# interpreting-video-features/interpreting-video-features

Hardware: AMD Instinct MI355X
Metric: clips/sec full mask-search (I3D, 16f, 300 iters) (higher is better)
Workload: dtype f32 (each operand as 3 bf16 planes = 24 significand bits, 6 MFMA passes, f32 accumulate, f32 storage); 1 GPU; I3D perturbation mask search, 300 iters, synthetic clips [32,3,16,224,224] per GPU per step (BASELINE configs[1]); init_mask + search + reverse score + Grad-CAM; iters=300, frames=16, math=bf16x6

## Files before the change

### interpreting-video-features_amd/csrc/conv3d_halo.hip

```cpp
#include "conv3d_halo_impl.h"

namespace ivf {

template int conv_halo_launch_variant_am<AM_X3>(ConvKArgs& a, int v, hipStream_t s);
extern template int conv_halo_launch_variant_am<AM_X6>(ConvKArgs& a, int v, hipStream_t s);
extern template int conv_halo_launch_variant_am<AM_BF16>(ConvKArgs& a, int v, hipStream_t s);

int conv_halo_supported(const ConvKArgs& a) {
  if (a.sT != 1 || a.sH != 1 || a.sW != 1) return 0;
  if (a.kT * a.kH * a.kW <= 1 || a.kT > 4 || a.kH > 4 || a.kW > 4) return 0;
  if (a.Cin % 8) return 0;
  return 1;
}

int conv_halo_num_variants() { return HALO_NUM_VARIANTS; }

int conv_halo_launch_variant(ConvKArgs& a, int math, int v, hipStream_t s) {
  switch (math) {
    case IVF_MATH_BF16X3: return conv_halo_launch_variant_am<AM_X3>(a, v, s);
    case IVF_MATH_BF16X6: return conv_halo_launch_variant_am<AM_X6>(a, v, s);
    case IVF_MATH_BF16ACT: return conv_halo_launch_variant_am<AM_BF16>(a, v, s);
  }
  set_error("conv3d_halo: arithmetic mode %d has no LDS-halo kernel", math);
  return IVF_ERR_UNSUPPORTED;
}

int conv_halo_launch(ConvKArgs& a, int math, hipStream_t s) {
  static const int widths[5] = {192, 128, 96, 64, 32};
  int best = 32, best_cost = 1 << 30;
  for (int w : widths) {
    int cost = cdiv(a.Cout, w) * (w + 40);
    if (cost < best_cost) { best_cost = cost; best = w; }
  }
  const bool deep = a.To >= 4;
  if (math == IVF_MATH_BF16X6) {
    switch (best) {
      case 192: return conv_halo_launch_variant(a, math, deep ? 68 : 18, s);
      case 128: return conv_halo_launch_variant(a, math, deep ? 61 : 9, s);
      case 96: return conv_halo_launch_variant(a, math, deep ? 20 : 10, s);
      case 64: return conv_halo_launch_variant(a, math, deep ? 21 : 11, s);
      default: return conv_halo_launch_variant(a, math, deep ? 37 : 12, s);
    }
  }
  switch (best) {
    case 192: return conv_halo_launch_variant(a, math, deep ? 0 : 8, s);
    case 128: return conv_halo_launch_variant(a, math, deep ? 1 : 9, s);
    case 96: return conv_halo_launch_variant(a, math, deep ? 3 : 10, s);
    case 64: return conv_halo_launch_variant(a, math, deep ? 5 : 11, s);
    default: return conv_halo_launch_variant(a, math, deep ? 7 : 12, s);
  }
}

}
```

### interpreting-video-features_amd/csrc/conv3d_halo_impl.h

```cpp
#pragma once
#include <algorithm>
#include <type_traits>

#include "conv_common.h"

namespace ivf {

#ifdef IVF_HALO_STAMPS
static __device__ unsigned long long g_halo_stamps[8];
#define IVF_STAMP(var) const unsigned long long var = __builtin_amdgcn_s_memtime()
#define IVF_STAMP_RT(var) const unsigned long long var = __builtin_amdgcn_s_memrealtime()
#define IVF_STAMP_ADD(slot, t1, t0) \
  do { if (threadIdx.x == 0) atomicAdd(&g_halo_stamps[slot], (t1) - (t0)); } while (0)
#else
#define IVF_STAMP(var) do {} while (0)
#define IVF_STAMP_RT(var) do {} while (0)
#define IVF_STAMP_ADD(slot, t1, t0) do {} while (0)
#endif

__device__ __forceinline__ void tile_hw(int p, int hw_pitch, int* h, int* w) {
  const int b0 = p & 1, b1 = (p >> 1) & 1, b2 = (p >> 2) & 1, b3 = (p >> 3) & 1, b4 = (p >> 4) & 1;
  const int half = p >> 5;
  int hl, ww;
  if (hw_pitch == 10) {
    ww = b0 | (b2 << 1) | (b1 << 2);
    hl = b3 | (b4 << 1);
  } else if (hw_pitch == 11) {
    ww = b0 | (b2 << 1) | (b3 << 2);
    hl = b1 | (b4 << 1);
  } else {
    ww = p & 7;
    hl = (p >> 3) & 3;
  }
  *h = half * 4 + hl;
  *w = ww;
}

template <int TT, int TH, int TW>
__device__ __forceinline__ void box_pos(int row, int hw_pitch, int* t, int* h, int* w) {
  if constexpr (TT == 4 && TW == 8) {
    const int li = row & 31, q = li >> 2, ql = q & 3;
    const int sel = ((ql + 1) >> 1) & 1;
    *t = (q >> 2) ? 3 - sel : sel;
    *w = (ql >> 1) * 4 + (li & 3);
    *h = row >> 5;
  } else if constexpr (TH == 8 && TW == 8) {
    tile_hw(row & 63, hw_pitch, h, w);
    *t = row >> 6;
  } else {
    const int p = row % (TH * TW);
    *t = row / (TH * TW);
    *h = p / TW;
    *w = p % TW;
  }
}

template <int TT, int TH, int TW>
__host__ __device__ constexpr int halo_plane_rows(int HH, int HW) {
  int ps = HH * HW;
  if (TT == 4 && TW == 8) ps += (4 - ps % 8 + 8) % 8;
  return ps;
}

template <int AM, int TT, int BN, int WROWS, int WCOLS, int KS, int BKH, int TH, int TW, int TPS, bool DMA>
__global__ __launch_bounds__((TT * TH * TW / WROWS) * (BN / WCOLS) * KS * 64) void conv3d_halo_kernel(ConvKArgs a,
                                                                                                int tilesT,
                                                                                                int tilesH,
                                                                                                int tilesW) {
  constexpr int BM = TT * TH * TW;
  constexpr int NPA = OpPlanes<AM>::A, NPB = OpPlanes<AM>::B;
  static_assert(BM % WROWS == 0 && WROWS % 32 == 0 && BN % WCOLS == 0 && WCOLS % 32 == 0, "tile");
  static_assert((KS * BN * (BKH / 8)) % 64 == 0, "weight-stream slots must fill whole waves");
  constexpr int WM = BM / WROWS, WN = BN / WCOLS;
  constexpr int NT = WM * WN * KS * 64;
  constexpr int TM = WROWS / 32, TN = WCOLS / 32;
  constexpr int ROWB = (BKH + 8) * 2;
  constexpr int ROWB_B = DMA ? BKH * 2 : ROWB;
  static_assert(!DMA || BKH == 32, "the LDS-DMA weight stream is written for 32-channel chunks");
  constexpr int G4 = BKH / 4;
  constexpr int G8 = BKH / 8;
  constexpr int BLOADS = (TPS * KS * BN * G8 + NT - 1) / NT;

  extern __shared__ __attribute__((aligned(16))) unsigned char smem[];
  IVF_STAMP(st_begin);
  IVF_STAMP_RT(rt_begin);
  const int HT = TT + a.kT - 1, HH = TH + a.kH - 1, HW = TW + a.kW - 1;
  const int PS = halo_plane_rows<TT, TH, TW>(HH, HW);
  const int HR = HT * PS;
  unsigned char* a_hi = smem;
  const size_t APL = (size_t)HR * ROWB;
  unsigned char* b_base = smem + (size_t)NPA * HR * ROWB;
  int* rowoff = reinterpret_cast<int*>(b_base + (size_t)2 * NPB * TPS * KS * BN * ROWB_B);

  const int tid = threadIdx.x;
  const int lane = tid & 63;
  const int wave = __builtin_amdgcn_readfirstlane(tid >> 6);
  const int wk = wave / (WM * WN);
  const int wm = (wave % (WM * WN)) / WN, wn = wave % WN;
  const int li = lane & 31, lh = lane >> 5;

  int tile = xcd_remap(blockIdx.x, gridDim.x);
  const int nt = tile % a.ntiles;
  tile /= a.ntiles;
  const int tw = tile % tilesW;
  tile /= tilesW;
  const int th = tile % tilesH;
  tile /= tilesH;
  const int tt = tile % tilesT;
  const int b = tile / tilesT;
  const int t0 = tt * TT, h0 = th * TH, w0 = tw * TW;
  const int n0 = nt * BN;

  int arow[TM];
#pragma unroll
  for (int i = 0; i < TM; ++i) {
    int r = wm * WROWS + i * 32 + li;
    int pt, ph, pw;
    box_pos<TT, TH, TW>(r, HW, &pt, &ph, &pw);
    arow[i] = pt * PS + ph * HW + pw;
  }
  const int ntaps = a.kT * a.kH * a.kW;
  const int ntg = (ntaps + KS - 1) / KS;
  const int nsteps = (ntg + TPS - 1) / TPS;
  const int khw = a.kH * a.kW;
  for (int row = tid; row < HR; row += NT) {
    int ht = row / PS;
    int rem = row - ht * PS;
    int hh = rem / HW;
    int hw = rem - hh * HW;
    int ti = t0 - a.pT + ht, hi = h0 - a.pH + hh, wi = w0 - a.pW + hw;
    bool ok = hh < HH && (unsigned)ti < (unsigned)a.Ti && (unsigned)hi < (unsigned)a.Hi && (unsigned)wi < (unsigned)a.Wi;
    rowoff[row] = ok ? ((b * a.Ti + ti) * a.Hi + hi) * a.Wi + wi : -1;
  }

  f32x16 acc[TM][TN];
#pragma unroll
  for (int i = 0; i < TM; ++i)
#pragma unroll
    for (int j = 0; j < TN; ++j)
#pragma unroll
      for (int r = 0; r < 16; ++r) acc[i][j][r] = 0.f;

  constexpr int PF = 3;
  typedef unsigned int u32x4 __attribute__((ext_vector_type(4)));
  u32x4 rb[PF][NPB][BLOADS] = {};
  int b_src[BLOADS];
  int b_dst[BLOADS];
  int b_tap[BLOADS];
  int b_c[BLOADS];
#pragma unroll
  for (int q = 0; q < BLOADS; ++q) {
    const int idx = tid + q * NT;
    const int sub = idx / (KS * BN * G8);
    const int r1 = idx - sub * (KS * BN * G8);
    const int grp = r1 / (BN * G8);
    const int rem = r1 - grp * (BN * G8);
    const int row = BKH == 32 ? perm8(rem / G8) : rem / G8, g2 = rem % G8;
    const int n = min(n0 + row, a.Cout - 1);
    b_src[q] = sub < TPS ? n * a.ldw : 0;
    b_dst[q] = sub < TPS ? ((sub * KS + grp) * NPB * BN + row) * ROWB_B + 16 * g2 : -1;
    b_tap[q] = sub < TPS ? sub + grp * ntg : 0;
    b_c[q] = 8 * g2;
  }
  auto load_b = [&](int slot, int step, int c0) __attribute__((always_inline)) {
    const int s0 = min(step, nsteps - 1) * TPS;
#pragma unroll
    for (int q = 0; q < BLOADS; ++q) {
      const int tap = min(s0 + b_tap[q], ntaps - 1);
      int c = c0 + b_c[q];
      c = c < a.Cin ? c : 0;
      const unsigned short* p = a.wbf + (size_t)(b_src[q] + tap * a.Cin + c);
      if (b_dst[q] >= 0) {
#pragma unroll
        for (int pl = 0; pl < NPB; ++pl) rb[slot][pl][q] = *reinterpret_cast<const u32x4*>(p + pl * a.w_lo_off);
      }
    }
  };
  auto store_b = [&](int slot, int buf) __attribute__((always_inline)) {
    unsigned char* bb = b_base + (size_t)buf * (TPS * KS * NPB * BN * ROWB_B);
#pragma unroll
    for (int q = 0; q < BLOADS; ++q) {
      if (b_dst[q] >= 0) {
#pragma unroll
        for (int pl = 0; pl < NPB; ++pl) *reinterpret_cast<u32x4*>(bb + b_dst[q] + pl * BN * ROWB_B) = rb[slot][pl][q];
      }
    }
  };
  int g_kw, g_kh, g_toff;
  {
    const int tap0 = wk * ntg;
    const int kt = tap0 / khw;
    const int rem = tap0 - kt * khw;
    g_kh = rem / a.kW;
    g_kw = rem - g_kh * a.kW;
    g_toff = (kt * PS + g_kh * HW + g_kw) * ROWB;
  }
  int t_kw = 0, t_kh = 0, t_off = 0;
  auto tap_advance = [&]() __attribute__((always_inline)) {
    t_off += ROWB;
    if (++t_kw == a.kW) {
      t_kw = 0;
      t_off += (HW - a.kW) * ROWB;
      if (++t_kh == a.kH) {
        t_kh = 0;
        t_off += (PS - a.kH * HW) * ROWB;
      }
    }
  };
  int abase[TM];
#pragma unroll
  for (int i = 0; i < TM; ++i) abase[i] = arow[i] * ROWB + 16 * lh;
  auto b_off = [&](int j, int ks) __attribute__((always_inline)) {
    const int row = wn * WCOLS + j * 32 + li;
    if constexpr (DMA) return row * ROWB_B + 16 * ((2 * ks + lh) ^ ((row >> 2) & 3));
    else return row * ROWB_B + ks * 32 + 16 * lh;
  };
  constexpr int NP = TPS * KS * NPB * BN * (BKH / 8), NI = NP / 64, NWV = NT / 64, MAXI = (NI + NWV - 1) / NWV;
  int d_base[MAXI], d_tap[MAXI], d_c[MAXI];
  if constexpr (DMA) {
#pragma unroll
    for (int k = 0; k < MAXI; ++k) {
      const int p = (wave + k * NWV) * 64 + lane;
      const int slot = p % G8, row = (p / G8) % BN, plane = (p / (G8 * BN)) % NPB;
      const int grp = (p / (G8 * BN * NPB)) % KS, sb = p / (G8 * BN * NPB * KS);
      d_base[k] = plane * (int)a.w_lo_off + min(n0 + row, a.Cout - 1) * a.ldw;
      d_tap[k] = sb + grp * ntg;
      d_c[k] = 8 * (slot ^ ((row >> 2) & 3));
    }
  }
  auto dma_b = [&](int step, int buf, int c0) __attribute__((always_inline)) {
    if constexpr (DMA) {
#pragma unroll
      for (int k = 0; k < MAXI; ++k) {
        if (wave + k * NWV >= NI) continue;
        const int tap = min(step * TPS + d_tap[k], ntaps - 1);
        int c = c0 + d_c[k];
        c = c < a.Cin ? c : 0;
        const unsigned short* g = a.wbf + (size_t)(d_base[k] + tap * a.Cin + c);
        unsigned char* dst = b_base + (size_t)buf * (TPS * KS * NPB * BN * ROWB_B) + (size_t)(wave + k * NWV) * 1024;
        __builtin_amdgcn_global_load_lds((const __attribute__((address_space(1))) void*)g,
                                         (__attribute__((address_space(3))) void*)dst, 16, 0, 0);
      }
    }
  };
  constexpr int NKS = BKH / 16;
  constexpr bool PIPELINED = (TM == 1 && TN == 1);
  auto mma_tap = [&](int step, int buf, int nks) __attribute__((always_inline)) {
    const int lt0 = step * TPS;
    const int nsub = min(TPS, min(ntg - lt0, ntaps - wk * ntg - lt0));
    if (nsub <= 0) return;
    const unsigned char* bstep = b_base + (size_t)(buf * TPS * KS + wk) * NPB * BN * ROWB_B;
    if constexpr (PIPELINED) {
      bf16x8 fa[2][NPA], fb[2][NPB];
      auto issue = [&](int slot, int sub, int ks) __attribute__((always_inline)) {
        const int aoff = abase[0] + t_off + ks * 32;
        const unsigned char* bh = bstep + (size_t)sub * KS * NPB * BN * ROWB_B + b_off(0, ks);
#pragma unroll
        for (int pl = 0; pl < NPA; ++pl) fa[slot][pl] = *reinterpret_cast<const bf16x8*>(a_hi + pl * APL + aoff);
#pragma unroll
        for (int pl = 0; pl < NPB; ++pl) fb[slot][pl] = *reinterpret_cast<const bf16x8*>(bh + (size_t)pl * BN * ROWB_B);
      };
      issue(0, 0, 0);
#pragma unroll
      for (int u = 0; u < TPS * NKS; ++u) {
        if (u / NKS < nsub) {
          if (u + 1 < TPS * NKS && (u + 1) / NKS < nsub) {
            if ((u + 1) % NKS == 0) tap_advance();
            issue((u + 1) & 1, (u + 1) / NKS, (u + 1) % NKS);
          }
          mma_planes<AM>(fa[u & 1], fb[u & 1], acc[0][0]);
          __builtin_amdgcn_sched_group_barrier(0x100, NPA + NPB, 0);
          __builtin_amdgcn_sched_group_barrier(0x008, AM == AM_X6 ? 6 : (AM == AM_BF16 ? 2 : 3), 0);
        }
      }
      tap_advance();
    } else {
#pragma unroll
      for (int sub = 0; sub < TPS; ++sub) {
        if (sub >= nsub) break;
        const unsigned char* bh = bstep + (size_t)sub * KS * NPB * BN * ROWB_B;
        for (int ks = 0; ks < nks; ++ks) {
          bf16x8 fa[TM][NPA];
#pragma unroll
          for (int i = 0; i < TM; ++i) {
            const int off = abase[i] + t_off + ks * 32;
#pragma unroll
            for (int pl = 0; pl < NPA; ++pl) fa[i][pl] = *reinterpret_cast<const bf16x8*>(a_hi + pl * APL + off);
          }
#pragma unroll
          for (int j = 0; j < TN; ++j) {
            const int off = b_off(j, ks);
            bf16x8 fb[NPB];
#pragma unroll
            for (int pl = 0; pl < NPB; ++pl) fb[pl] = *reinterpret_cast<const bf16x8*>(bh + (size_t)pl * BN * ROWB_B + off);
#pragma unroll
            for (int i = 0; i < TM; ++i) mma_planes<AM>(fa[i], fb, acc[i][j]);
          }
        }
        tap_advance();
      }
    }
  };

  constexpr int NSTG = 4;
  float4 stg[NSTG];
  const int ngroups = BKH == 32 ? ((HR + 7) & ~7) * G4 : HR * G4;
  int stage_base = 0;
  auto stage_load = [&](int c0) __attribute__((always_inline)) {
#pragma unroll
    for (int u = 0; u < NSTG; ++u) {
      int idx = stage_base + u * NT + tid;
      float4 v = make_float4(0.f, 0.f, 0.f, 0.f);
      if (idx < ngroups) {
        int row = BKH == 32 ? perm8(idx / G4) : idx / G4, g = idx % G4;
        if (row >= HR) row = -1;
        int c = c0 + 4 * g;
        int pos = row >= 0 ? rowoff[row] : -1;
        if (pos >= 0 && c < a.Cin) v = load_act4<AM>(a.in, (size_t)pos * a.in_ld + a.in_coff + c);
      }
      stg[u] = v;
    }
  };
  auto stage_store = [&]() __attribute__((always_inline)) {
#pragma unroll
    for (int u = 0; u < NSTG; ++u) {
      int idx = stage_base + u * NT + tid;
      const int srow = BKH == 32 ? perm8(idx / G4) : idx / G4;
      if (idx < ngroups && srow < HR) {
        stage_planes<AM>(a_hi + srow * ROWB + 8 * (idx % G4), APL, stg[u]);
      }
    }
  };
  __syncthreads();

  for (int c0 = 0; c0 < a.Cin; c0 += BKH) {
    if constexpr (!DMA) {
      load_b(0, 0, c0);
      load_b(1, 1, c0);
      load_b(2, 2, c0);
    }
    __syncthreads();
    dma_b(0, 0, c0);
    IVF_STAMP(st_s0);
    for (stage_base = 0; stage_base < ngroups; stage_base += NSTG * NT) {
      stage_load(c0);
      stage_store();
    }
    stage_base = 0;
    __builtin_amdgcn_s_waitcnt(0x0F70);
    if constexpr (!DMA) store_b(0, 0);
    __syncthreads();
    IVF_STAMP(st_s1);
    IVF_STAMP_ADD(1, st_s1, st_s0);

    const int cw = min(BKH, a.Cin - c0);
    const int nks = (cw + 15) >> 4;
    t_kw = g_kw, t_kh = g_kh, t_off = g_toff;
    auto tap_body = [&](auto U, int tap0) __attribute__((always_inline)) {
      constexpr int u = decltype(U)::value;
      const int tap = tap0 + u;
      load_b(u, tap + PF, c0);
      if (tap < nsteps) mma_tap(tap, tap & 1, nks);
      store_b((u + 1) % PF, (tap + 1) & 1);
      __syncthreads();
    };
    static_assert(PF == 3, "tap loop is unrolled by hand for a 3-deep ring");
    if constexpr (DMA) {
      for (int tap = 0; tap < nsteps; ++tap) {
        if (tap + 1 < nsteps) dma_b(tap + 1, (tap + 1) & 1, c0);
        mma_tap(tap, tap & 1, nks);
        asm volatile("s_waitcnt vmcnt(0)" ::: "memory");
        __syncthreads();
      }
    } else {
      for (int tap0 = 0; tap0 < nsteps; tap0 += PF) {
        tap_body(std::integral_constant<int, 0>{}, tap0);
        tap_body(std::integral_constant<int, 1>{}, tap0);
        tap_body(std::integral_constant<int, 2>{}, tap0);
      }
    }
    IVF_STAMP(st_s2);
    IVF_STAMP_ADD(2, st_s2, st_s1);
  }
  IVF_STAMP(st_loop_end);

  if constexpr (KS == 2) {
    float* red = reinterpret_cast<float*>(smem);
    const int slot = (wm * WN + wn) * TM * TN;
    if (wk == 1) {
#pragma unroll
      for (int i = 0; i < TM; ++i)
#pragma unroll
        for (int j = 0; j < TN; ++j)
#pragma unroll
          for (int r = 0; r < 16; ++r) red[((slot + i * TN + j) * 16 + r) * 64 + lane] = acc[i][j][r];
    }
    __syncthreads();
    if (wk == 0) {
#pragma unroll
      for (int i = 0; i < TM; ++i)
#pragma unroll
        for (int j = 0; j < TN; ++j)
#pragma unroll
          for (int r = 0; r < 16; ++r) acc[i][j][r] += red[((slot + i * TN + j) * 16 + r) * 64 + lane];
    }
    __syncthreads();
  }

  if (TH == 8 && TW == 8 && BN == 32 && a.d2s && a.Cout == 32 && a.bsT == 2 && a.bsH == 2 && a.bsW == 2 && !a.accumulate && !a.relu &&
      a.dC == 4 && (a.out_ld & 3) == 0 && (a.out_coff & 3) == 0) {
    float* ot = reinterpret_cast<float*>(smem);
    if (wk == 0) {
      const int n = wn * WCOLS + li;
      const int par = n >> 2, c = n & 3;
      const int pt = par >> 2, ph = (par >> 1) & 1, pw = par & 1;
#pragma unroll
      for (int i = 0; i < TM; ++i)
#pragma unroll
        for (int r = 0; r < 16; ++r) {
          const int row = wm * WROWS + i * 32 + (r & 3) + 8 * (r >> 2) + 4 * lh;
          int bt, bh, bw;
          box_pos<TT, TH, TW>(row, HW, &bt, &bh, &bw);
          const int tt2 = 2 * bt + pt, hh2 = 2 * bh + ph, ww2 = 2 * bw + pw;
          ot[((tt2 * 16 + hh2) * 16 + ww2) * 4 + c] = acc[i][0][r];
        }
    }
    __syncthreads();
    for (int p = tid; p < 2 * TT * 256; p += NT) {
      const int t = 2 * t0 + (p >> 8), h = 2 * h0 + ((p >> 4) & 15), w = 2 * w0 + (p & 15);
      if (t < a.dT && h < a.dH && w < a.dW)
        *reinterpret_cast<float4*>(a.out + ((size_t)((b * a.dT + t) * a.dH + h) * a.dW + w) * a.out_ld + a.out_coff) =
            *reinterpret_cast<const float4*>(ot + (size_t)p * 4);
    }
    IVF_STAMP(st_end_d2s);
    IVF_STAMP_RT(rt_end_d2s);
    IVF_STAMP_ADD(5, rt_end_d2s, rt_begin);
    IVF_STAMP_ADD(3, st_end_d2s, st_loop_end);
    IVF_STAMP_ADD(0, st_end_d2s, st_begin);
    IVF_STAMP_ADD(4, st_begin + 1, st_begin);
    return;
  }
  if (wk != 0) return;

  conv_epilogue<AM, TM, TN>(
      a, acc,
      [&](int row) {
        int pt, ph, pw;
        box_pos<TT, TH, TW>(row, HW, &pt, &ph, &pw);
        int t = t0 + pt, h = h0 + ph, w = w0 + pw;
        if (t >= a.To || h >= a.Ho || w >= a.Wo) return -1;
        return ((b * a.To + t) * a.Ho + h) * a.Wo + w;
      },
      wm * WROWS, n0 + wn * WCOLS, li, lh);
  IVF_STAMP(st_end);
  IVF_STAMP_RT(rt_end);
  IVF_STAMP_ADD(5, rt_end, rt_begin);
  IVF_STAMP_ADD(3, st_end, st_loop_end);
  IVF_STAMP_ADD(0, st_end, st_begin);
  IVF_STAMP_ADD(4, st_begin + 1, st_begin);
}

#if defined(IVF_HALO_STAMPS) && defined(IVF_HALO_STAMPS_OWNER)
}
extern "C" int ivf_debug_halo_stamps(unsigned long long* out8, int reset) {
  IVF_CHECK_HIP(hipMemcpyFromSymbol(out8, HIP_SYMBOL(ivf::g_halo_stamps), 8 * sizeof(unsigned long long)));
  if (reset) {
    unsigned long long z[8] = {0};
    IVF_CHECK_HIP(hipMemcpyToSymbol(HIP_SYMBOL(ivf::g_halo_stamps), z, sizeof(z)));
  }
  return IVF_OK;
}
namespace ivf {
#endif

template <int AM, int TT, int BN, int WROWS, int WCOLS, int KS = 1, int BKH = 32, int TH = 8, int TW = 8, int TPS = 1, bool DMA = false>
static int launch_halo(ConvKArgs& a, int variant_id, hipStream_t s) {
  constexpr int NPA = OpPlanes<AM>::A, NPB = OpPlanes<AM>::B;
  constexpr int NT = (TT * TH * TW / WROWS) * (BN / WCOLS) * KS * 64;
  constexpr int ROWB = (BKH + 8) * 2;
  constexpr int ROWB_B = DMA ? BKH * 2 : ROWB;
  const int HR = (TT + a.kT - 1) * halo_plane_rows<TT, TH, TW>(TH + a.kH - 1, TW + a.kW - 1);
  size_t shm = (size_t)NPA * HR * ROWB + (size_t)2 * TPS * KS * NPB * BN * ROWB_B + (size_t)HR * sizeof(int);
  if (KS == 2) shm = std::max(shm, (size_t)TT * TH * TW * BN * 4);
  if (a.d2s) shm = std::max(shm, (size_t)2 * TT * 256 * 4 * sizeof(float));
  if (shm > 160 * 1024) {
    set_error("conv3d_halo: %zu bytes of LDS needed", shm);
    return IVF_ERR_UNSUPPORTED;
  }
  static LdsAttrOnce once;
  IVF_PROPAGATE(raise_lds_limit(reinterpret_cast<const void*>(&conv3d_halo_kernel<AM, TT, BN, WROWS, WCOLS, KS, BKH, TH, TW, TPS, DMA>), 160 * 1024, once));
  const int tilesT = cdiv(a.To, TT), tilesH = cdiv(a.Ho, TH), tilesW = cdiv(a.Wo, TW);
  a.ntiles = cdiv(a.Cout, BN);
  a.mtiles = a.B * tilesT * tilesH * tilesW;
  dim3 grid(a.mtiles * a.ntiles);
  prof_name(IVF_CONV_HALO_BASE + variant_id, "conv3d_halo_kernel<%d,%d,%d,%d,%d,%d,%d,%d,%d,%d,%s>", AM, TT, BN, WROWS, WCOLS, KS,
            BKH, TH, TW, TPS, DMA ? "true" : "false");
  const bool timed = prof_begin(s, IVF_CONV_HALO_BASE + variant_id);
  hipLaunchKernelGGL((conv3d_halo_kernel<AM, TT, BN, WROWS, WCOLS, KS, BKH, TH, TW, TPS, DMA>), grid, dim3(NT), shm, s, a, tilesT, tilesH, tilesW);
  if (timed) prof_end(s);
  IVF_CHECK_LAUNCH();
  return IVF_OK;
}


constexpr int HALO_NUM_VARIANTS = 70;

template <int AM, int TT, int BN, int KS, int BKH, int TH, int TW, int TPS, bool DMA>
constexpr bool halo_variant_built() {
  constexpr int ROWB = (BKH + 8) * 2, ROWB_B = DMA ? BKH * 2 : ROWB;
  constexpr int HH = TH + 2, HW = TW + 2;
  constexpr int PS = HH * HW + ((TT == 4 && TW == 8) ? (4 - (HH * HW) % 8 + 8) % 8 : 0);
  constexpr long HR = (long)(TT + 2) * PS;
  constexpr long shm = OpPlanes<AM>::A * HR * ROWB + 2L * TPS * KS * OpPlanes<AM>::B * BN * ROWB_B + HR * 4;
  return shm <= 160 * 1024;
}
template <int AM, int TT, int BN, int WROWS, int WCOLS, int KS = 1, int BKH = 32, int TH = 8, int TW = 8, int TPS = 1, bool DMA = false>
static int launch_halo_if(ConvKArgs& a, int variant_id, hipStream_t s) {
  if constexpr (halo_variant_built<AM, TT, BN, KS, BKH, TH, TW, TPS, DMA>()) {
    return launch_halo<AM, TT, BN, WROWS, WCOLS, KS, BKH, TH, TW, TPS, DMA>(a, variant_id, s);
  } else {
    set_error("conv3d_halo: variant %d needs more than 160 KB of LDS in this arithmetic mode", variant_id);
    return IVF_ERR_UNSUPPORTED;
  }
}

template <int AM>
int conv_halo_launch_variant_am(ConvKArgs& a, int v, hipStream_t s) {
  switch (v) {
    case 0: return launch_halo_if<AM, 4, 192, 32, 96>(a, 0, s);
    case 1: return launch_halo_if<AM, 4, 128, 64, 64>(a, 1, s);
    case 2: return launch_halo_if<AM, 4, 128, 32, 64>(a, 2, s);
    case 3: return launch_halo_if<AM, 4, 96, 32, 96>(a, 3, s);
    case 4: return launch_halo_if<AM, 4, 64, 32, 64>(a, 4, s);
    case 5: return launch_halo_if<AM, 4, 64, 64, 64, 2>(a, 5, s);
    case 6: return launch_halo_if<AM, 4, 32, 32, 32>(a, 6, s);
    case 7: return launch_halo_if<AM, 4, 32, 64, 32, 2>(a, 7, s);
    case 8: return launch_halo_if<AM, 2, 192, 32, 96>(a, 8, s);
    case 9: return launch_halo_if<AM, 2, 128, 32, 64>(a, 9, s);
    case 10: return launch_halo_if<AM, 2, 96, 32, 96>(a, 10, s);
    case 11: return launch_halo_if<AM, 2, 64, 32, 64>(a, 11, s);
    case 12: return launch_halo_if<AM, 2, 32, 32, 32>(a, 12, s);
    case 13: return launch_halo_if<AM, 2, 64, 64, 64, 2>(a, 13, s);
    case 14: return launch_halo_if<AM, 2, 128, 64, 64>(a, 14, s);
    case 15: return launch_halo_if<AM, 4, 64, 32, 64, 2>(a, 15, s);
    case 16: return launch_halo_if<AM, 4, 96, 32, 96, 2>(a, 16, s);
    case 17: return launch_halo_if<AM, 4, 32, 32, 32, 2>(a, 17, s);
    case 18: return launch_halo_if<AM, 2, 192, 32, 96, 1, 16>(a, 18, s);
    case 19: return launch_halo_if<AM, 2, 128, 32, 64, 1, 16>(a, 19, s);
    case 20: return launch_halo_if<AM, 4, 96, 32, 96, 1, 16>(a, 20, s);
    case 21: return launch_halo_if<AM, 4, 64, 32, 64, 1, 16>(a, 21, s);
    case 22: return launch_halo_if<AM, 2, 96, 32, 96, 1, 16>(a, 22, s);
    case 23: return launch_halo_if<AM, 4, 192, 32, 96, 1, 32, 4, 14>(a, 23, s);
    case 24: return launch_halo_if<AM, 4, 128, 32, 64, 1, 32, 4, 14>(a, 24, s);
    case 25: return launch_halo_if<AM, 4, 96, 32, 96, 1, 32, 4, 14>(a, 25, s);
    case 26: return launch_halo_if<AM, 4, 64, 32, 64, 1, 32, 4, 14>(a, 26, s);
    case 27: return launch_halo_if<AM, 4, 32, 32, 32, 1, 32, 4, 14>(a, 27, s);
    case 28: return launch_halo_if<AM, 4, 64, 32, 32, 1, 32, 4, 14>(a, 28, s);
    case 29: return launch_halo_if<AM, 4, 32, 32, 32, 2, 32, 4, 14>(a, 29, s);
    case 30: return launch_halo_if<AM, 4, 128, 32, 128, 1, 32, 4, 14>(a, 30, s);
    case 31: return launch_halo_if<AM, 2, 32, 64, 32, 2, 16>(a, 31, s);
    case 32: return launch_halo_if<AM, 2, 32, 32, 32, 2, 16>(a, 32, s);
    case 33: return launch_halo_if<AM, 2, 32, 32, 32, 1, 16>(a, 33, s);
    case 34: return launch_halo_if<AM, 2, 64, 32, 64, 2, 16>(a, 34, s);
    case 35: return launch_halo_if<AM, 2, 64, 64, 64, 2, 16>(a, 35, s);
    case 36: return launch_halo_if<AM, 4, 32, 64, 32, 2, 16>(a, 36, s);
    case 37: return launch_halo_if<AM, 4, 32, 32, 32, 2, 16>(a, 37, s);
    case 38: return launch_halo_if<AM, 4, 32, 32, 32, 2, 16, 8, 8, 4>(a, 38, s);
    case 39: return launch_halo_if<AM, 4, 32, 64, 32, 2, 16, 8, 8, 4>(a, 39, s);
    case 40: return launch_halo_if<AM, 4, 32, 32, 32, 2, 16, 8, 8, 2>(a, 40, s);
    case 41: return launch_halo_if<AM, 2, 32, 32, 32, 2, 32, 8, 8, 2>(a, 41, s);
    case 42: return launch_halo_if<AM, 4, 64, 32, 64, 1, 16, 8, 8, 2>(a, 42, s);
    case 43: return launch_halo_if<AM, 4, 64, 32, 64, 1, 32, 8, 8, 2>(a, 43, s);
    case 44: return launch_halo_if<AM, 4, 32, 32, 32, 1, 16, 8, 8, 4>(a, 44, s);
    case 45: return launch_halo_if<AM, 4, 96, 32, 96, 1, 16, 8, 8, 2>(a, 45, s);
    case 46: return launch_halo_if<AM, 4, 32, 32, 32, 2, 32, 8, 8, 2>(a, 46, s);
    case 47: return launch_halo_if<AM, 4, 64, 32, 64, 1, 32, 4, 14, 2>(a, 47, s);
    case 48: return launch_halo_if<AM, 4, 192, 32, 96, 1, 32, 7, 8>(a, 48, s);
    case 49: return launch_halo_if<AM, 4, 128, 32, 64, 1, 32, 7, 8>(a, 49, s);
    case 50: return launch_halo_if<AM, 4, 96, 32, 96, 1, 16, 7, 8>(a, 50, s);
    case 51: return launch_halo_if<AM, 4, 64, 32, 64, 1, 16, 7, 8>(a, 51, s);
    case 52: return launch_halo_if<AM, 4, 192, 32, 96, 1, 32, 8, 8, 1, true>(a, 52, s);
    case 53: return launch_halo_if<AM, 4, 192, 32, 96, 1, 32, 4, 14, 1, true>(a, 53, s);
    case 54: return launch_halo_if<AM, 4, 128, 32, 64, 1, 32, 4, 14, 1, true>(a, 54, s);
    case 55: return launch_halo_if<AM, 4, 128, 32, 64, 1, 32, 8, 8, 1, true>(a, 55, s);
    case 56: return launch_halo_if<AM, 4, 32, 32, 32, 2, 32, 8, 8, 1, true>(a, 56, s);
    case 57: return launch_halo_if<AM, 4, 128, 32, 64, 1, 32, 7, 8, 1, true>(a, 57, s);
    case 58: return launch_halo_if<AM, 4, 96, 32, 96, 1, 32, 8, 8, 1, true>(a, 58, s);
    case 59: return launch_halo_if<AM, 4, 64, 32, 64, 1, 32, 8, 8, 1, true>(a, 59, s);
    case 60: return launch_halo_if<AM, 4, 192, 32, 96, 1, 16>(a, 60, s);
    case 61: return launch_halo_if<AM, 4, 128, 32, 64, 1, 16>(a, 61, s);
    case 62: return launch_halo_if<AM, 4, 192, 32, 96, 1, 16, 4, 14>(a, 62, s);
    case 63: return launch_halo_if<AM, 4, 128, 32, 64, 1, 16, 4, 14>(a, 63, s);
    case 64: return launch_halo_if<AM, 4, 96, 32, 96, 1, 16, 4, 14>(a, 64, s);
    case 65: return launch_halo_if<AM, 4, 64, 32, 64, 1, 16, 4, 14>(a, 65, s);
    case 66: return launch_halo_if<AM, 4, 192, 32, 96, 1, 16, 7, 8>(a, 66, s);
    case 67: return launch_halo_if<AM, 4, 128, 32, 64, 1, 16, 7, 8>(a, 67, s);
    case 68: return launch_halo_if<AM, 4, 192, 64, 96, 1, 16>(a, 68, s);
    case 69: return launch_halo_if<AM, 4, 128, 64, 64, 1, 16>(a, 69, s);
  }
  set_error("conv3d_halo: unknown variant %d", v);
  return IVF_ERR_BAD_ARG;
}

}
```

### interpreting-video-features_amd/csrc/ivf_common.hip

```cpp
#include <cstring>

#include "ivf_common.h"

namespace ivf {
static thread_local char g_err[512] = "";
void set_error(const char* fmt, ...) {
  va_list ap;
  va_start(ap, fmt);
  vsnprintf(g_err, sizeof(g_err), fmt, ap);
  va_end(ap);
}
}

extern "C" const char* ivf_last_error(void) { return ivf::g_err; }
extern "C" int ivf_version(void) { return 301; }

#include <vector>
namespace ivf {
struct Prof {
  bool enabled = false, active = false;
  int every = 1;
  size_t cap = 0, used = 0;
  std::vector<hipEvent_t> ev;
  std::vector<int> variant;
  std::vector<int> site;
  std::vector<double> flops;
  double next_flops = 0.0;
  int next_site = -1;
};
static Prof g_prof;
static char g_prof_names[IVF_PROFILE_CLASSES][96];
void prof_name(int variant, const char* fmt, ...) {
  if (variant < 0 || variant >= IVF_PROFILE_CLASSES) return;
  va_list ap;
  va_start(ap, fmt);
  vsnprintf(g_prof_names[variant], sizeof(g_prof_names[variant]), fmt, ap);
  va_end(ap);
}
void prof_set_iteration(int it) { g_prof.active = g_prof.enabled && it >= 0 && (it % g_prof.every == 0); }
void prof_set_flops(double f) { g_prof.next_flops = f; }
void prof_set_site(int site) { g_prof.next_site = site; }
bool prof_begin(hipStream_t s, int variant) {
  Prof& p = g_prof;
  if (!p.active || p.used >= p.cap) return false;
  if (p.ev.size() < 2 * (p.used + 1)) {
    hipEvent_t a, b;
    if (hipEventCreate(&a) != hipSuccess || hipEventCreate(&b) != hipSuccess) return false;
    p.ev.push_back(a);
    p.ev.push_back(b);
  }
  p.variant.resize(p.used + 1);
  p.site.resize(p.used + 1);
  p.flops.resize(p.used + 1);
  p.variant[p.used] = variant;
  p.site[p.used] = p.next_site;
  p.flops[p.used] = p.next_flops;
  (void)hipEventRecord(p.ev[2 * p.used], s);
  return true;
}
void prof_end(hipStream_t s) {
  Prof& p = g_prof;
  (void)hipEventRecord(p.ev[2 * p.used + 1], s);
  p.used++;
}
}

extern "C" int ivf_profile_enable(int every, int max_launches) {
  IVF_CHECK_ARG(every >= 1 && max_launches > 0, "profile_enable: bad args");
  ivf::g_prof.enabled = true;
  ivf::g_prof.active = false;
  ivf::g_prof.every = every;
  ivf::g_prof.cap = (size_t)max_launches;
  ivf::g_prof.used = 0;
  return IVF_OK;
}

extern "C" int ivf_profile_disable(void) {
  ivf::g_prof.enabled = false;
  ivf::g_prof.active = false;
  return IVF_OK;
}

extern "C" const char* ivf_profile_class_name(int cls) {
  return (cls >= 0 && cls < IVF_PROFILE_CLASSES) ? ivf::g_prof_names[cls] : "";
}

extern "C" int ivf_profile_collect_sites(double* kernel_ms, long long* launches, double* flops, int* variant,
                                         int max_sites) {
  IVF_CHECK_ARG(kernel_ms && launches && flops && variant && max_sites > 0, "profile_collect_sites: bad args");
  ivf::Prof& p = ivf::g_prof;
  for (int v = 0; v < max_sites; ++v) { kernel_ms[v] = 0.0; launches[v] = 0; flops[v] = 0.0; variant[v] = -1; }
  for (size_t i = 0; i < p.used; ++i) {
    const int st = p.site[i];
    if (st < 0 || st >= max_sites) continue;
    IVF_CHECK_HIP(hipEventSynchronize(p.ev[2 * i + 1]));
    float ms = 0.f;
    IVF_CHECK_HIP(hipEventElapsedTime(&ms, p.ev[2 * i], p.ev[2 * i + 1]));
    kernel_ms[st] += ms;
    launches[st] += 1;
    flops[st] += p.flops[i];
    variant[st] = p.variant[i];
  }
  return IVF_OK;
}

extern "C" int ivf_profile_collect(double* kernel_ms, long long* launches, double* flops) {
  IVF_CHECK_ARG(kernel_ms && launches && flops, "profile_collect: null pointer");
  ivf::Prof& p = ivf::g_prof;
  for (int v = 0; v < IVF_PROFILE_CLASSES; ++v) { kernel_ms[v] = 0.0; launches[v] = 0; flops[v] = 0.0; }
  for (size_t i = 0; i < p.used; ++i) {
    IVF_CHECK_HIP(hipEventSynchronize(p.ev[2 * i + 1]));
    float ms = 0.f;
    IVF_CHECK_HIP(hipEventElapsedTime(&ms, p.ev[2 * i], p.ev[2 * i + 1]));
    int v = p.variant[i];
    if (v < 0 || v >= IVF_PROFILE_CLASSES) continue;
    kernel_ms[v] += ms;
    launches[v] += 1;
    flops[v] += p.flops[i];
  }
  p.used = 0;
  return IVF_OK;
}
```

Baseline: 3.926 clips/s.

## Add raster-row halo conv variant for 3x3x3 convs on 14x14 maps

Adds a new conv3d halo kernel mode (RP=15) that tiles the output as a flat run of 256 consecutive output positions in raster order. The input halo is staged as a padded 15x15-pitch raster window, so each tap becomes a constant row offset and unpadded LDS rows are used. The dispatcher routes bf16x6 3x3x3 padding-1 convs on 13-14 spatial maps with Cout >= 2*Cin to this variant. The aim is to remove the wasted work and halo overhead that 8x8 box tiles incur on 14x14 maps. In exchange it stages a larger, irregular halo window per block and skips the LDS row padding, which may add bank conflicts.

Result: no change. 3.934 clips/s, median of 6 (+0.2%).

```diff
diff --git a/interpreting-video-features_amd/csrc/conv3d_halo.hip b/interpreting-video-features_amd/csrc/conv3d_halo.hip
--- a/interpreting-video-features_amd/csrc/conv3d_halo.hip
+++ b/interpreting-video-features_amd/csrc/conv3d_halo.hip
@@ -34,6 +34,9 @@
   }
   const bool deep = a.To >= 4;
   if (math == IVF_MATH_BF16X6) {
+    if (a.kT == 3 && a.kH == 3 && a.kW == 3 && a.pT == 1 && a.pH == 1 && a.pW == 1 && !a.d2s && a.Ho >= 13 && a.Ho <= 14 &&
+        a.Wo >= 13 && a.Wo <= 14 && a.Cin >= 144 && a.Cout >= 2 * a.Cin)
+      return conv_halo_launch_variant(a, math, 70, s);
     switch (best) {
       case 192: return conv_halo_launch_variant(a, math, deep ? 68 : 18, s);
       case 128: return conv_halo_launch_variant(a, math, deep ? 61 : 9, s);
diff --git a/interpreting-video-features_amd/csrc/conv3d_halo_impl.h b/interpreting-video-features_amd/csrc/conv3d_halo_impl.h
--- a/interpreting-video-features_amd/csrc/conv3d_halo_impl.h
+++ b/interpreting-video-features_amd/csrc/conv3d_halo_impl.h
@@ -62,7 +62,23 @@
   return ps;
 }
 
-template <int AM, int TT, int BN, int WROWS, int WCOLS, int KS, int BKH, int TH, int TW, int TPS, bool DMA>
+template <int RP>
+__host__ __device__ inline int raster_x(int m, int T, int H, int W) {
+  const int w = m % W;
+  const int r1 = m / W;
+  const int h = r1 % H;
+  const int r2 = r1 / H;
+  const int t = r2 % T, b = r2 / T;
+  return (b * (T + 1) + t + 1) * RP * RP + (h + 1) * RP + (w + 1);
+}
+template <int RP>
+inline int raster_window_bound(int BM, int T, int H, int W) {
+  const int steps = BM - 1;
+  const int span = steps + cdiv(steps, W) * (RP - W) + cdiv(steps, H * W) * (RP * RP - H * RP) + cdiv(steps, T * H * W) * RP * RP;
+  return span + 2 * (RP * RP + RP + 1) + 1;
+}
+
+template <int AM, int TT, int BN, int WROWS, int WCOLS, int KS, int BKH, int TH, int TW, int TPS, bool DMA, int RP = 0>
 __global__ __launch_bounds__((TT * TH * TW / WROWS) * (BN / WCOLS) * KS * 64) void conv3d_halo_kernel(ConvKArgs a,
                                                                                                 int tilesT,
                                                                                                 int tilesH,
@@ -74,8 +90,8 @@
   constexpr int WM = BM / WROWS, WN = BN / WCOLS;
   constexpr int NT = WM * WN * KS * 64;
   constexpr int TM = WROWS / 32, TN = WCOLS / 32;
-  constexpr int ROWB = (BKH + 8) * 2;
-  constexpr int ROWB_B = DMA ? BKH * 2 : ROWB;
+  constexpr int ROWB = RP ? BKH * 2 : (BKH + 8) * 2;
+  constexpr int ROWB_B = DMA ? BKH * 2 : (BKH + 8) * 2;
   static_assert(!DMA || BKH == 32, "the LDS-DMA weight stream is written for 32-channel chunks");
   constexpr int G4 = BKH / 4;
   constexpr int G8 = BKH / 8;
@@ -84,12 +100,20 @@
   extern __shared__ __attribute__((aligned(16))) unsigned char smem[];
   IVF_STAMP(st_begin);
   IVF_STAMP_RT(rt_begin);
-  const int HT = TT + a.kT - 1, HH = TH + a.kH - 1, HW = TW + a.kW - 1;
-  const int PS = halo_plane_rows<TT, TH, TW>(HH, HW);
-  const int HR = HT * PS;
+  static_assert(RP == 0 || (KS == 1 && !DMA), "raster rows: one tap group, register weight stream");
+  const int HT = TT + a.kT - 1, HH = TH + a.kH - 1, HW = RP ? RP : TW + a.kW - 1;
+  const int PS = RP ? RP * RP : halo_plane_rows<TT, TH, TW>(HH, HW);
+  int m0 = 0, m1 = 0, x0 = 0;
+  if constexpr (RP > 0) {
+    m0 = (xcd_remap(blockIdx.x, gridDim.x) / a.ntiles) * BM;
+    m1 = min(m0 + BM, a.M) - 1;
+    x0 = raster_x<RP>(m0, a.To, a.Ho, a.Wo) - (PS + HW + 1);
+  }
+  const int HRA = RP ? tilesT : HT * PS;
+  const int HR = RP ? min(raster_x<RP>(m1, a.To, a.Ho, a.Wo) - x0 + PS + HW + 2, HRA) : HRA;
   unsigned char* a_hi = smem;
-  const size_t APL = (size_t)HR * ROWB;
-  unsigned char* b_base = smem + (size_t)NPA * HR * ROWB;
+  const size_t APL = (size_t)HRA * ROWB;
+  unsigned char* b_base = smem + (size_t)NPA * HRA * ROWB;
   int* rowoff = reinterpret_cast<int*>(b_base + (size_t)2 * NPB * TPS * KS * BN * ROWB_B);
 
   const int tid = threadIdx.x;
@@ -115,15 +139,28 @@
 #pragma unroll
   for (int i = 0; i < TM; ++i) {
     int r = wm * WROWS + i * 32 + li;
-    int pt, ph, pw;
-    box_pos<TT, TH, TW>(r, HW, &pt, &ph, &pw);
-    arow[i] = pt * PS + ph * HW + pw;
+    if constexpr (RP > 0) {
+      arow[i] = raster_x<RP>(min(m0 + r, m1), a.To, a.Ho, a.Wo) - (x0 + PS + HW + 1);
+    } else {
+      int pt, ph, pw;
+      box_pos<TT, TH, TW>(r, HW, &pt, &ph, &pw);
+      arow[i] = pt * PS + ph * HW + pw;
+    }
   }
   const int ntaps = a.kT * a.kH * a.kW;
   const int ntg = (ntaps + KS - 1) / KS;
   const int nsteps = (ntg + TPS - 1) / TPS;
   const int khw = a.kH * a.kW;
   for (int row = tid; row < HR; row += NT) {
+    if constexpr (RP > 0) {
+      const int x = x0 + row;
+      const int e = x / PS - 1, q = x - (e + 1) * PS;
+      const int bb = e / (a.Ti + 1), ti = e - bb * (a.Ti + 1);
+      const int hi = q / HW - 1, wi = q % HW - 1;
+      const bool ok = e >= 0 && ti < a.Ti && bb < a.B && (unsigned)hi < (unsigned)a.Hi && (unsigned)wi < (unsigned)a.Wi;
+      rowoff[row] = ok ? ((bb * a.Ti + ti) * a.Hi + hi) * a.Wi + wi : -1;
+      continue;
+    }
     int ht = row / PS;
     int rem = row - ht * PS;
     int hh = rem / HW;
@@ -445,6 +482,7 @@
   conv_epilogue<AM, TM, TN>(
       a, acc,
       [&](int row) {
+        if constexpr (RP > 0) return m0 + row <= m1 ? m0 + row : -1;
         int pt, ph, pw;
         box_pos<TT, TH, TW>(row, HW, &pt, &ph, &pw);
         int t = t0 + pt, h = h0 + ph, w = w0 + pw;
@@ -473,13 +511,19 @@
 namespace ivf {
 #endif
 
-template <int AM, int TT, int BN, int WROWS, int WCOLS, int KS = 1, int BKH = 32, int TH = 8, int TW = 8, int TPS = 1, bool DMA = false>
+template <int AM, int TT, int BN, int WROWS, int WCOLS, int KS = 1, int BKH = 32, int TH = 8, int TW = 8, int TPS = 1, bool DMA = false, int RP = 0>
 static int launch_halo(ConvKArgs& a, int variant_id, hipStream_t s) {
   constexpr int NPA = OpPlanes<AM>::A, NPB = OpPlanes<AM>::B;
   constexpr int NT = (TT * TH * TW / WROWS) * (BN / WCOLS) * KS * 64;
-  constexpr int ROWB = (BKH + 8) * 2;
-  constexpr int ROWB_B = DMA ? BKH * 2 : ROWB;
-  const int HR = (TT + a.kT - 1) * halo_plane_rows<TT, TH, TW>(TH + a.kH - 1, TW + a.kW - 1);
+  constexpr int ROWB = RP ? BKH * 2 : (BKH + 8) * 2;
+  constexpr int ROWB_B = DMA ? BKH * 2 : (BKH + 8) * 2;
+  if (RP > 0 && !(a.kT == 3 && a.kH == 3 && a.kW == 3 && a.pT == 1 && a.pH == 1 && a.pW == 1 && !a.d2s && a.Ti == a.To &&
+                  a.Hi == a.Ho && a.Wi == a.Wo && a.Ho < RP && a.Wo < RP)) {
+    set_error("conv3d_halo: raster-row variant %d serves 3x3x3 / padding 1 on maps up to %d x %d", variant_id, RP - 1, RP - 1);
+    return IVF_ERR_UNSUPPORTED;
+  }
+  const int HR = RP > 0 ? raster_window_bound<(RP > 0 ? RP : 1)>(TT * TH * TW, a.To, a.Ho, a.Wo)
+                        : (TT + a.kT - 1) * halo_plane_rows<TT, TH, TW>(TH + a.kH - 1, TW + a.kW - 1);
   size_t shm = (size_t)NPA * HR * ROWB + (size_t)2 * TPS * KS * NPB * BN * ROWB_B + (size_t)HR * sizeof(int);
   if (KS == 2) shm = std::max(shm, (size_t)TT * TH * TW * BN * 4);
   if (a.d2s) shm = std::max(shm, (size_t)2 * TT * 256 * 4 * sizeof(float));
@@ -488,22 +532,26 @@
     return IVF_ERR_UNSUPPORTED;
   }
   static LdsAttrOnce once;
-  IVF_PROPAGATE(raise_lds_limit(reinterpret_cast<const void*>(&conv3d_halo_kernel<AM, TT, BN, WROWS, WCOLS, KS, BKH, TH, TW, TPS, DMA>), 160 * 1024, once));
-  const int tilesT = cdiv(a.To, TT), tilesH = cdiv(a.Ho, TH), tilesW = cdiv(a.Wo, TW);
+  IVF_PROPAGATE(raise_lds_limit(reinterpret_cast<const void*>(&conv3d_halo_kernel<AM, TT, BN, WROWS, WCOLS, KS, BKH, TH, TW, TPS, DMA, RP>), 160 * 1024, once));
+  const int tilesT = RP > 0 ? HR : cdiv(a.To, TT), tilesH = RP > 0 ? 1 : cdiv(a.Ho, TH), tilesW = RP > 0 ? 1 : cdiv(a.Wo, TW);
   a.ntiles = cdiv(a.Cout, BN);
-  a.mtiles = a.B * tilesT * tilesH * tilesW;
+  a.mtiles = RP > 0 ? cdiv(a.M, TT * TH * TW) : a.B * tilesT * tilesH * tilesW;
   dim3 grid(a.mtiles * a.ntiles);
-  prof_name(IVF_CONV_HALO_BASE + variant_id, "conv3d_halo_kernel<%d,%d,%d,%d,%d,%d,%d,%d,%d,%d,%s>", AM, TT, BN, WROWS, WCOLS, KS,
-            BKH, TH, TW, TPS, DMA ? "true" : "false");
+  if (RP > 0)
+    prof_name(IVF_CONV_HALO_BASE + variant_id, "conv3d_halo_kernel<%d,%d,%d,%d,%d,%d,%d,%d,%d,%d,%s,%d>", AM, TT, BN, WROWS, WCOLS,
+              KS, BKH, TH, TW, TPS, DMA ? "true" : "false", RP);
+  else
+    prof_name(IVF_CONV_HALO_BASE + variant_id, "conv3d_halo_kernel<%d,%d,%d,%d,%d,%d,%d,%d,%d,%d,%s>", AM, TT, BN, WROWS, WCOLS, KS,
+              BKH, TH, TW, TPS, DMA ? "true" : "false");
   const bool timed = prof_begin(s, IVF_CONV_HALO_BASE + variant_id);
-  hipLaunchKernelGGL((conv3d_halo_kernel<AM, TT, BN, WROWS, WCOLS, KS, BKH, TH, TW, TPS, DMA>), grid, dim3(NT), shm, s, a, tilesT, tilesH, tilesW);
+  hipLaunchKernelGGL((conv3d_halo_kernel<AM, TT, BN, WROWS, WCOLS, KS, BKH, TH, TW, TPS, DMA, RP>), grid, dim3(NT), shm, s, a, tilesT, tilesH, tilesW);
   if (timed) prof_end(s);
   IVF_CHECK_LAUNCH();
   return IVF_OK;
 }
 
 
-constexpr int HALO_NUM_VARIANTS = 70;
+constexpr int HALO_NUM_VARIANTS = 72;
 
 template <int AM, int TT, int BN, int KS, int BKH, int TH, int TW, int TPS, bool DMA>
 constexpr bool halo_variant_built() {
@@ -597,6 +645,8 @@
     case 67: return launch_halo_if<AM, 4, 128, 32, 64, 1, 16, 7, 8>(a, 67, s);
     case 68: return launch_halo_if<AM, 4, 192, 64, 96, 1, 16>(a, 68, s);
     case 69: return launch_halo_if<AM, 4, 128, 64, 64, 1, 16>(a, 69, s);
+    case 70: return launch_halo<AM, 1, 64, 32, 64, 1, 16, 1, 256, 1, false, 15>(a, 70, s);
+    case 71: return launch_halo<AM, 1, 128, 32, 64, 1, 16, 1, 256, 1, false, 15>(a, 71, s);
   }
   set_error("conv3d_halo: unknown variant %d", v);
   return IVF_ERR_BAD_ARG;
diff --git a/interpreting-video-features_amd/csrc/ivf_common.hip b/interpreting-video-features_amd/csrc/ivf_common.hip
--- a/interpreting-video-features_amd/csrc/ivf_common.hip
+++ b/interpreting-video-features_amd/csrc/ivf_common.hip
@@ -13,7 +13,7 @@
 }
 
 extern "C" const char* ivf_last_error(void) { return ivf::g_err; }
-extern "C" int ivf_version(void) { return 301; }
+extern "C" int ivf_version(void) { return 302; }
 
 #include <vector>
 namespace ivf {
```
